# AdeeshKolluru/AdsorbDiff

Hardware: AMD Instinct MI355X
Metric: sampled adsorbate sites/sec (50 denoise steps, ~200-atom slabs) (higher is better)
Workload: dtype f32 (f16x3-split MFMA, fp32 accumulate; ADF_GEMM=f32 selects exact f32)

## Files before the change

### adsorbdiff_amd/csrc/api.hip

```cpp
#include <stdarg.h>
#include <stdlib.h>
#include <string.h>

#include <new>

#include "common.h"

static thread_local char g_err[512] = "";

void adf_set_error(const char* fmt, ...) {
    va_list ap;
    va_start(ap, fmt);
    vsnprintf(g_err, sizeof(g_err), fmt, ap);
    va_end(ap);
}

extern "C" const char* adf_last_error(void) { return g_err; }
extern "C" const char* adf_version(void) { return "adsorbdiff_hip 0.5.0 (gfx950)"; }

adf_tune adf_tune_from_env() {
    auto off_is_0 = [](const char* name) { const char* e = getenv(name); return (e && atoi(e) == 0) ? 0 : 1; };
    auto is_f32 = [](const char* name) { const char* e = getenv(name); return e && strcmp(e, "f32") == 0; };
    adf_tune t = {};
    const char* mi = getenv("ADF_GEMM16_MI");
// ... 5 lines not shown
    t.gemm_wr_fused = wf ? atoi(wf) : 2;
    if (t.gemm_wr_fused != 0 && t.gemm_wr_fused != 4) t.gemm_wr_fused = 2;
    t.head_gate_fused = off_is_0("ADF_HEAD_GATE_FUSED");
    t.lift_emit = off_is_0("ADF_LIFT_EMIT");
    t.graph_sys_csr = off_is_0("ADF_GRAPH_SYS_CSR");
    t.train_gemm16 = is_f32("ADF_TRAIN_GEMM") ? 0 : 1;
    t.wgrad_f32 = is_f32("ADF_WGRAD") ? 1 : 0;
    const char* pw = getenv("ADF_EQV2_PW_MI");
    t.eqv2_pw_mi = (pw && atoi(pw) == 3) ? 3 : 4;
    const char* gt = getenv("ADF_EQV2_GEMM_TILE");
    t.eqv2_gemm_tile256 = (gt && atoi(gt) == 128) ? 0 : 1;
    t.eqv2_rotin_generic = getenv("ADF_EQV2_ROTIN_GENERIC") != nullptr;
    t.eqv2_rotout_generic = getenv("ADF_EQV2_ROTOUT_GENERIC") != nullptr;
    const char* r4 = getenv("ADF_GEMM_ROWS4");
    t.gemm_rows4 = r4 ? (atoi(r4) & 3) : 3;
    return t;
}
const adf_tune& adf_tune_process() {
    static const adf_tune t = adf_tune_from_env();
    return t;
}
int adf_current_num_cus() {
    int dev = 0, n = 0;
    if (hipGetDevice(&dev) != hipSuccess || hipDeviceGetAttribute(&n, hipDeviceAttributeMultiprocessorCount, dev) != hipSuccess) return 0;
    return n;
}

extern "C" int32_t adf_profile_enable(adf_painn_t h, int32_t on) {
    if (!h) { adf_set_error("null handle"); return ADF_EINVAL; }
    h->prof.enable(on != 0);
// ... 377 lines not shown
    const bool lift = h->lift_on && !h->gemm_f32;
    const bool em = lift && h->tune.lift_emit;
    ADF_TRY(adf_nodewise_layernorm(x, w.ln_w, w.ln_b, h->y, n, H, s, em ? h->mag_a : nullptr, h->rows_dev));
    ADF_TRY(adf_linear(h, h->y, H, w.xp0_w, &w.xp0_16, w.xp0_b, h->cat, H, n, H, H, 1, s, em ? h->mag_a : nullptr,
                       em ? h->mag_b : nullptr));
    if (h->gemm_f32) {
        if (row_map) { adf_set_error("internal: mapped records need the f16x3 path"); return ADF_EINVAL; }
        ADF_TRY(adf_launch_gemm(h->cat, H, w.xp2_w, H, w.xp2_b, h->xh, 3 * H, n, 3 * H, H, 0, s));
        ADF_TRY(adf_pack_records(h, n, h->xh, vec, vec_is_zero, s, rec));
    } else {
        adf_epi ep = {};
        ep.vec_in = vec; ep.rec = rec ? rec : h->rec; ep.H = H; ep.vec_is_zero = vec_is_zero ? 1 : 0;
        ep.row_map = row_map;
        ep.rmag = em ? h->mag_b : nullptr;
        ep.m_dev = h->rows_dev;
        ADF_TRY(adf_launch_gemm16_fused(h->cat, H, &w.xp2_16, n, H, H, 1, &ep, s, h->tune, lift ? &h->lift : nullptr));
    }
    adf_prof_end(h, s);
    return ADF_OK;
}

static int32_t message_layer(adf_painn* h, int l, int N, const float* x, const float* vec, float* x_out,
                             float* vec_out, bool vec_is_zero, hipStream_t s, const int32_t* tlist = nullptr,
                             int n_targets = 0, float* rec = nullptr, bool records_ready = false) {
    if (!records_ready) ADF_TRY(make_records(h, l, N, x, vec, vec_is_zero, rec, nullptr, s));
    adf_prof_begin(h, ADF_PROF_MESSAGE, s);
    const int items = tlist ? n_targets : N;
    const bool emit = h->rmx && h->lift_on && !h->gemm_f32 && !h->msg_f32 && items > 0 && items <= h->part_stride;
    h->part_x = h->part_vec = nullptr;
    const int32_t st = adf_message_impl(h, l, N, x, h->xh, vec, x_out, vec_out, vec_is_zero, s, tlist, n_targets, rec,
                                        tlist ? h->rows_dev : nullptr, emit ? h->xpart : nullptr, h->vpart, h->part_stride);
// ... 39 lines not shown
        adf_epi e0 = {};
        e0.A2 = h->cat; e0.K1 = H; e0.m_dev = h->rows_dev;
        e0.rmag = parts ? h->lift.buf : nullptr;
        e0.out_mag = h->lift_on ? reinterpret_cast<unsigned int*>(h->mag_b) : nullptr;
        ADF_TRY(adf_launch_gemm16(x, H, &w.xv0_16, w.xv0_b, h->y, H, N, H, 2 * H, 1, &e0, s, lf, h->tune, h->num_cus));
    }
    int32_t st;
    if (h->gemm_f32) {
        ADF_TRY(adf_launch_gemm(h->y, H, w.xv2_w, H, w.xv2_b, h->xh, 3 * H, N, 3 * H, H, 0, s));
        st = adf_nodewise_update_apply(h->xh, h->dot, h->vv, x, vec, h->scale[l], N, H, s);
    } else {
        adf_epi ep = {};
        ep.x = x; ep.vec = vec; ep.dot = h->dot; ep.vv = h->vv; ep.scale = h->scale[l]; ep.H = H;
        ep.rmag = h->lift_on ? h->mag_b : nullptr;
        ep.m_dev = h->rows_dev;
        st = adf_launch_gemm16_fused(h->y, H, &w.xv2_16, N, H, H, 2, &ep, s, h->tune);
    }
    adf_prof_end(h, s);
    return st;
}

extern "C" int32_t adf_painn_message_layer(adf_painn_t h, int32_t layer, int32_t N, const float* x, const float* vec,
                                           float* x_out, float* vec_out, void* stream) {
    if (!h || !h->weights_set || layer < 0 || layer >= h->hp.num_layers || N != h->lastN) {
        adf_set_error("message_layer: bad handle/layer, or N differs from the built graph");
        return ADF_EINVAL;
    }
    hipStream_t s = (hipStream_t)stream;
    ADF_TRY(zero_pad_rows(h, N, s));
    ADF_TRY(message_layer(h, layer, N, x, vec, x_out, vec_out, false, s));
    return ADF_OK;
}

extern "C" int32_t adf_painn_update_layer(adf_painn_t h, int32_t layer, int32_t N, float* x, float* vec, void* stream) {
    if (!h || !h->weights_set || layer < 0 || layer >= h->hp.num_layers) {
        adf_set_error("update_layer: bad handle/layer");
        return ADF_EINVAL;
    }
    ADF_TRY(ensure_capacity(h, N, 1));
    return update_layer(h, layer, N, x, vec, (hipStream_t)stream, false);
}

extern "C" int32_t adf_painn_get_tune(adf_painn_t h, adf_tune* out) {
    if (!h || !out) { adf_set_error("get_tune: null handle or output"); return ADF_EINVAL; }
    *out = h->tune;
    return ADF_OK;
}

extern "C" int32_t adf_painn_debug_row_maxima(adf_painn_t h, int32_t which, float* out, int64_t capacity, int32_t* rows,
                                              void* stream) {
    if (!h || which < 0 || which > 6) { adf_set_error("debug_row_maxima: null handle or which outside 0..6"); return ADF_EINVAL; }
    if (which == 4) { h->dbg_capture = capacity != 0; h->dbg_comb_rows = 0; return ADF_OK; }
    const int H = h->hp.hidden_channels, ns = H / ADF_SLICE_CH;
    const int n = which <= 1 ? h->dbg_msg_rows : which <= 3 ? h->dbg_cat_rows : h->dbg_comb_rows;
    if (!h->rmx_part || n <= 0) { adf_set_error("debug_row_maxima: no launch has emitted row maxima (ADF_ROW_MAXIMA=0?)"); return ADF_EINVAL; }
    if (rows) *rows = n;
    if (!out) return ADF_OK;
    const int64_t need = (which == 1 || which == 5) ? 3ll * n : which == 3 ? (int64_t)n * H : n;
    if (capacity < need) { adf_set_error("debug_row_maxima: out holds %lld floats, need %lld", (long long)capacity, (long long)need); return ADF_EINVAL; }
    hipStream_t s = (hipStream_t)stream;
// ... 516 lines not shown
```

### adsorbdiff_amd/csrc/common.h

```cpp
#pragma once
#include <hip/hip_runtime.h>
#include <stdint.h>
#include <stdio.h>
#include <string>
#include <vector>

#include "../../include/adsorbdiff_hip.h"

#define ADF_GROUP_NODES 32
#define ADF_SLICE_CH 64
#define ADF_MAX_CAND 1024
#define ADF_MAX_K 128
#define ADF_NFLAGS 8
#define ADF_MAX_INDEG 1024
#define ADF_MAX_LAYERS 16

void adf_set_error(const char* fmt, ...);

#define ADF_HIP_CHECK(expr)                                                             \
    do {                                                                                \
        hipError_t _e = (expr);                                                         \
        if (_e != hipSuccess) {                                                         \
            adf_set_error("%s failed: %s (%s:%d)", #expr, hipGetErrorString(_e),        \
                          __FILE__, __LINE__);                                          \
// ... 260 lines not shown
const adf_tune& adf_tune_process();
int adf_current_num_cus();
int32_t adf_launch_gemm16(const float* A, int lda, const adf_w16* W, const float* bias, float* C, int ldc, int M,
                          int N, int K, int act_ssilu, const adf_epi* ep, hipStream_t s, const adf_lift* lf,
                          const adf_tune& tune, int num_cus);
int32_t adf_launch_rowmag(const float* A, int lda, int K1, const float* A2, int K2, long long M, float* mag, hipStream_t s,
                          const int32_t* m_dev = nullptr, int m_mul = 1);
int32_t adf_launch_rowmax_combine(const float* part, long long stride, int nparts, long long M, float* mag, hipStream_t s,
                                  const int32_t* m_dev = nullptr, int m_mul = 1);
int32_t adf_split_weight(const float* w, long long n, adf_w16* out, unsigned int* scratch_bits, hipStream_t s,
                         int perm_H = 0, int K = 0, const float* bias = nullptr, int parts = 3);
int32_t adf_launch_gemm16_vecnorm(const float* A, int lda, const adf_w16* W, float* nrm, int M, int N, int K,
                                  hipStream_t s, const adf_tune& tune, const adf_lift* lf = nullptr,
                                  const float* premag = nullptr);
int32_t adf_launch_gemm16_fused(const float* A, int lda, const adf_w16* W, int M, int H, int K, int epi,
                                const adf_epi* ep, hipStream_t s, const adf_tune& tune, const adf_lift* lf = nullptr);
static inline int32_t adf_linear(const adf_painn* h, const float* A, int lda, const float* W, const adf_w16* W16,
                                 const float* bias, float* C, int ldc, int M, int N, int K, int act, hipStream_t s,
                                 const float* premag = nullptr, float* out_mag = nullptr) {
    if (h->gemm_f32) return adf_launch_gemm(A, lda, W, K, bias, C, ldc, M, N, K, act, s);
    adf_epi ep = {};
    ep.m_dev = h->rows_dev;
    if (h->lift_on) { ep.rmag = premag; ep.out_mag = reinterpret_cast<unsigned int*>(out_mag); }
    return adf_launch_gemm16(A, lda, W16, bias, C, ldc, M, N, K, act, &ep, s, h->lift_on ? &h->lift : nullptr, h->tune,
                             h->num_cus);
}
int32_t adf_pack_frag(const adf_w16* w, int N, int K, void* out, hipStream_t s);
int32_t adf_graph_build_impl(adf_painn* h, const adf_batch* b, hipStream_t s);
int32_t adf_energy_sum(const float* y, int H2, const float* w, const float* bias, const int32_t* atom_offset, float* energy,
                       int num_systems, hipStream_t s);
__device__ __forceinline__ float adf_row16_max(float v) {
// ... 95 lines not shown
```

### adsorbdiff_amd/csrc/gemm16.hip

```cpp
#include <stdlib.h>

#include "common.h"

typedef float f32x16 __attribute__((ext_vector_type(16)));
typedef _Float16 half8 __attribute__((ext_vector_type(8)));
typedef _Float16 half4 __attribute__((ext_vector_type(4)));

#ifndef EPI_ABL
#define EPI_ABL 0
#endif
#ifndef EPI2_POLICY
#define EPI2_POLICY 0
#endif
#ifndef G16_ABL
#define G16_ABL 0
#endif
#ifndef G16_WDEEP
#define G16_WDEEP 1
#endif
#ifndef G16_START_DELAY
#define G16_START_DELAY 0
#endif
#define HK 32
#define TLD3 96
// ... 2 lines not shown

__device__ __forceinline__ float adf_pow2_lift(float mx) {
    if (!(mx > 0.f) || !(mx < 3.0e38f)) return 1.0f;
    int e;
    (void)frexpf(mx, &e);
    e = 15 - e;
    e = e > 120 ? 120 : (e < -120 ? -120 : e);
    return ldexpf(1.0f, e);
}

__device__ __forceinline__ float ssilu16(float x) {
    float s = x / (1.0f + expf(-x));
    return s * 1.6666666666666667f;
}

template <int ACT, int MI, int NJ, int EPI, bool WR = false, int NWN = 2, int NWM = 2>
__global__ __launch_bounds__(64 * NWM * NWN, (MI == 4 || NWM * NWN == 8 ? 1 : 2)) void adf_gemm_f16x3_kernel(
    const float* __restrict__ A, int lda, const _Float16* __restrict__ Whi, const _Float16* __restrict__ Wlo,
    const float* __restrict__ inv_scale, const float* __restrict__ bias, float* __restrict__ C, int ldc, int Mh, int N,
    int K, int tiles_n, adf_epi ep) {
    const int M = ep.m_dev ? min(Mh, (int)*ep.m_dev) : Mh;
    static_assert(NWN == 2 || WR, "eight waves only with the register-streamed weights");
    static_assert(NWM == 2 || (NWM == 1 && WR), "one wave along M only with the register-streamed weights");
    constexpr int NT = 64 * NWM * NWN;
    constexpr int TM = 32 * MI * NWM;
    constexpr int TN = 32 * NJ * NWN;
    constexpr int NA = TM * 8 / NT;
    static_assert(TM * 8 % NT == 0, "A staging: whole float4s per thread");
    constexpr int LDS_WR = 4 * TM * HLD > NT / 64 * 6400 ? 4 * TM * HLD : NT / 64 * 6400;
    constexpr int LDS_MAIN = WR ? LDS_WR : (2 * TM + 2 * TN) * HLD;
    constexpr int LDS_REC = EPI == 1 ? NT / 64 * 2048 : 0;
    __shared__ __attribute__((aligned(16))) _Float16 lds[LDS_MAIN + LDS_REC];
    __shared__ float rinv[TM];
    _Float16* Ahi = lds;
    _Float16* Alo = Ahi + TM * HLD;
    _Float16* Bhi = Alo + TM * HLD;
    _Float16* Blo = Bhi + TN * HLD;
    const int tid = threadIdx.x;
    const int lane = tid & 63;
    const int wave = tid >> 6;
    const int wm = (wave / NWN) * (32 * MI);
    const int wn = (wave % NWN) * (32 * NJ);

    const int id = blockIdx.x;
    const int xcd = id & 7;
    const int qd = id >> 3;
    const int tile_m = (qd / tiles_n) * 8 + xcd;
    const int tile_n = qd % tiles_n;
    const int m0 = tile_m * (EPI >= 3 ? TM / 3 : TM);
    const int n0 = tile_n * TN;
    if (m0 >= M) return;
#if G16_START_DELAY
    if constexpr (NWM == 1) {
        if (qd >= 32 && qd < 64)
            for (int i = 0; i < G16_START_DELAY; ++i) __builtin_amdgcn_s_sleep(127);
    }
#endif

    unsigned int a_goff[NA];
    int a_off[NA];
    float a_rs[NA];
    auto global_row = [&](int row) -> unsigned int {
        if constexpr (EPI >= 3) {
            const int atom = m0 + (row / 96) * 32 + (row & 31), ax = (row % 96) >> 5;
            return (unsigned int)min(atom, M - 1) * 3u + ax;
        } else {
            return (unsigned int)min(m0 + row, M - 1);
        }
// ... 369 lines not shown
                const float a = acc[0][j][r] * (isc * rinv[wm + lr]), b = acc[1][j][r] * (isc * rinv[wm + 32 + lr]),
                            d = acc[2][j][r] * (isc * rinv[wm + 64 + lr]);
                T[lr * TLD2 + j * 32 + q] = sqrtf(a * a + b * b + d * d);
            }
        }
        __builtin_amdgcn_fence(__ATOMIC_RELEASE, "wavefront");
        __builtin_amdgcn_wave_barrier();
#pragma unroll
        for (int it = 0; it < 8; ++it) {
            const int lr = it * 4 + (lane >> 4), c4 = lane & 15;
            const int n = a0 + lr, c = cb + 4 * c4;
            if (n < M && c < N)
                *reinterpret_cast<float4*>(ep.cat + (size_t)n * N + c) = *reinterpret_cast<const float4*>(T + lr * TLD2 + 4 * c4);
        }
    } else {
        static_assert(EPI >= 3 || (NJ == 3 && MI == 2), "fused epilogues are written for the 64 x 96 wave tile");
        if (((EPI_ABL & 1) && EPI == 1) || ((EPI_ABL & 2) && EPI == 2)) {
            float sacc = 0.f;
            for (int i = 0; i < MI; ++i) for (int j = 0; j < NJ; ++j) for (int r = 0; r < 16; ++r) sacc += acc[i][j][r];
            if (ep.H < 0) ep.x[0] = sacc;
            return;
        }
        const int q = lane & 31;
        const int g = (n0 + wn) / 96;
        const int H = ep.H;
        const float b0 = bias[n0 + wn + q], b1 = bias[n0 + wn + 32 + q], b2 = bias[n0 + wn + 64 + q];
        __syncthreads();
        float* T = reinterpret_cast<float*>(lds) + wave * 3200;
#pragma unroll
        for (int i = 0; i < MI; ++i) {
#pragma unroll
// ... 109 lines not shown
                        for (int ax = 0; ax < 3; ++ax) {
                            float4 t = tv[it][ax];
                            const float4 v1 = w1[it][ax];
                            t.x += p2.x * v1.x; t.y += p2.y * v1.y; t.z += p2.z * v1.z; t.w += p2.w * v1.w;
                            EPI2_ST(rv, vr + ax * H, ep.vec, t);
                        }
                    }
#undef EPI2_ST
                }
            }
            __builtin_amdgcn_wave_barrier();
        }
    }
}

__global__ __launch_bounds__(256) void adf_rowmag_kernel(const float* __restrict__ A, int lda, int K1,
                                                         const float* __restrict__ A2, int K2, long long M,
                                                         float* __restrict__ mag, const int32_t* __restrict__ m_dev,
                                                         int m_mul) {
    const long long r = (long long)blockIdx.x * 4 + (threadIdx.x >> 6);
    const int lane = threadIdx.x & 63;
    if (r >= M || (m_dev && r >= (long long)*m_dev * m_mul)) return;
    float mx = 0.f;
    const float* a = A + (size_t)r * lda;
    for (int k = lane * 4; k < K1; k += 256) {
        const float4 v = *reinterpret_cast<const float4*>(a + k);
        mx = fmaxf(fmaxf(fmaxf(mx, fabsf(v.x)), fabsf(v.y)), fmaxf(fabsf(v.z), fabsf(v.w)));
    }
    if (A2) {
        const float* b = A2 + (size_t)r * lda;
// ... 100 lines not shown
        const long long cs = i >> 7;
        const int s = (int)(cs % nks), cb = (int)(cs / nks);
        const _Float16* src = (plane ? lo : hi) + (size_t)(32 * cb + (lane & 31)) * K + 16 * s + 8 * (lane >> 5);
        out[i] = *reinterpret_cast<const half8*>(src);
    }
}

int32_t adf_pack_frag(const adf_w16* w, int N, int K, void* out, hipStream_t s) {
    if (N % 32 || K % 16) { adf_set_error("pack_frag: N %% 32 or K %% 16"); return ADF_EINVAL; }
    hipLaunchKernelGGL(adf_pack_frag_kernel, dim3(256), dim3(256), 0, s, (const _Float16*)w->hi, (const _Float16*)w->lo,
                       (half8*)out, N, K);
    ADF_HIP_CHECK(hipGetLastError());
    return ADF_OK;
}

static int32_t check_a_span(long long rows, int lda) {
    if (rows * (long long)lda * 4 >= (1ll << 32)) {
        adf_set_error("gemm16: A operand of %lld rows x %d exceeds the 32-bit offset range, split the batch", rows, lda);
        return ADF_EOOM;
    }
    return ADF_OK;
}

int32_t adf_launch_gemm16(const float* A, int lda, const adf_w16* W, const float* bias, float* C, int ldc, int M,
                          int N, int K, int act_ssilu, const adf_epi* ep_in, hipStream_t s, const adf_lift* lf,
                          const adf_tune& tune, int num_cus) {
    if (M <= 0) return ADF_OK;
    adf_epi ep = {};
    if (ep_in) ep = *ep_in;
    if (!ep.A2) ep.K1 = 0;
// ... 7 lines not shown
    const int tiles_n = (N + TN - 1) / TN;
    const int tiles_m = (M + TM - 1) / TM;
    const int tiles_m8 = (tiles_m + 7) / 8 * 8;
    dim3 grid((unsigned)(tiles_m8 * tiles_n));
    if (ep.gate && (((N | ldc | ep.gate_ld) & 3) || (((uintptr_t)C | (uintptr_t)ep.gate) & 15))) {
        adf_set_error("gemm16: the gate epilogue needs N, ldc and gate_ld multiples of 4 and 16-byte aligned C and gate");
        return ADF_EINVAL;
    }
    ADF_TRY(lift_mags(A, lda, ep.A2 ? ep.K1 : K, ep.A2, ep.A2 ? K - ep.K1 : 0, M, lf, ep.rmag, &ep.rmag, s, ep.m_dev, 1));
    if (ep.out_mag) ADF_HIP_CHECK(hipMemsetAsync(ep.out_mag, 0, sizeof(float) * (size_t)M, s));
    const int ncu = num_cus > 0 ? num_cus : 256;
    const long long wg8 = (long long)((M + 191) / 192) * (N / 256 > 0 ? N / 256 : 1);
    const bool ragged = wg8 < 4ll * ncu && wg8 % ncu != 0 && wg8 % ncu < (3 * ncu) / 10 && wg8 > ncu;
    const long long wg4 = (long long)((M + 95) / 96) * (N / 256 > 0 ? N / 256 : 1), slots4 = 2ll * ncu;
    const bool ragged4 = wg4 < 4 * slots4 && wg4 % slots4 != 0 && wg4 % slots4 < (3 * slots4) / 10 && wg4 > slots4;
    if ((tune.gemm_rows4 & 1) && tune.gemm_w8_plain && W->frag && N % 256 == 0 && (K / HK) % 2 == 0 && mi == 2 && !ragged4) {
        const int tn4 = N / 256, tmw4 = ((M + 95) / 96 + 7) / 8 * 8;
        dim3 g4((unsigned)(tmw4 * tn4));
        if (act_ssilu)
            hipLaunchKernelGGL((adf_gemm_f16x3_kernel<1, 3, 2, 0, true, 4, 1>), g4, dim3(256), 0, s, A, lda, (const _Float16*)W->frag,
                               (const _Float16*)nullptr, W->inv_scale, bias, C, ldc, M, N, K, tn4, ep);
        else
            hipLaunchKernelGGL((adf_gemm_f16x3_kernel<0, 3, 2, 0, true, 4, 1>), g4, dim3(256), 0, s, A, lda, (const _Float16*)W->frag,
                               (const _Float16*)nullptr, W->inv_scale, bias, C, ldc, M, N, K, tn4, ep);
        ADF_HIP_CHECK(hipGetLastError());
        return ADF_OK;
    }
    if (!(tune.gemm_rows4 & 1) && tune.gemm_w8_plain && W->frag && N % 256 == 0 && (K / HK) % 2 == 0 && mi == 2 && !ragged) {
        const int tn8 = N / 256, tmw8 = ((M + 191) / 192 + 7) / 8 * 8;
        dim3 g8((unsigned)(tmw8 * tn8));
// ... 37 lines not shown
    if (tune.gemm_w8 && W->frag && N % 256 == 0 && (K / HK) % 2 == 0) {
        hipLaunchKernelGGL((adf_gemm_f16x3_kernel<0, 3, 2, 4, true, 4>), dim3((unsigned)(tm8 * (N / 256))), dim3(512), 0, s, A, lda,
                           (const _Float16*)W->frag, (const _Float16*)nullptr, W->inv_scale, (const float*)nullptr,
                           (float*)nullptr, 0, M, N, K, N / 256, ep);
        ADF_HIP_CHECK(hipGetLastError());
        return ADF_OK;
    }
    hipLaunchKernelGGL((adf_gemm_f16x3_kernel<0, 3, 2, 4>), dim3((unsigned)(tm8 * tn)), dim3(256), 0, s, A, lda,
                       (const _Float16*)W->hi, (const _Float16*)W->lo, W->inv_scale, (const float*)nullptr,
                       (float*)nullptr, 0, M, N, K, tn, ep);
    ADF_HIP_CHECK(hipGetLastError());
    return ADF_OK;
}

int32_t adf_launch_gemm16_fused(const float* A, int lda, const adf_w16* W, int M, int H, int K, int epi,
                                const adf_epi* ep_in, hipStream_t s, const adf_tune& tune, const adf_lift* lf) {
    adf_epi epv = *ep_in;
    const adf_epi* ep = &epv;
    if (M <= 0) return ADF_OK;
    if (K % HK != 0 || (lda & 3) || H % 64 != 0 || (epi != 3 && !W->bias_perm)) {
        adf_set_error("gemm16_fused: bad shape");
        return ADF_EINVAL;
    }
    ADF_TRY(check_a_span(epi == 3 ? 3ll * M : (long long)M, lda));
    ADF_TRY(lift_mags(A, lda, K, nullptr, 0, epi == 3 ? 3ll * M : (long long)M, lf, ep_in->rmag, &epv.rmag, s, ep_in->m_dev,
                      epi == 3 ? 3 : 1));
    const int N = 3 * H, TM = 128, TN = 192;
    const int tiles_n = N / TN;
    const int tiles_m = (M + TM - 1) / TM;
    const int tiles_m8 = (tiles_m + 7) / 8 * 8;
    dim3 grid((unsigned)(tiles_m8 * tiles_n));
// ... 3 lines not shown
            hipLaunchKernelGGL((adf_gemm_f16x3_kernel<0, 3, 2, 3, true, 4, 1>), dim3((unsigned)(((M + 31) / 32 + 7) / 8 * 8 * (2 * H / 256))),
                               dim3(256), 0, s, A, lda, (const _Float16*)W->frag, (const _Float16*)nullptr, W->inv_scale,
                               (const float*)nullptr, (float*)nullptr, 0, M, 2 * H, K, 2 * H / 256, *ep);
        else if (tune.gemm_wreg && W->frag && tune.gemm_w8 && (2 * H) % 256 == 0 && (K / HK) % 2 == 0)
            hipLaunchKernelGGL((adf_gemm_f16x3_kernel<0, 3, 2, 3, true, 4>), dim3((unsigned)(tm8 * (2 * H / 256))), dim3(512), 0, s,
                               A, lda, (const _Float16*)W->frag, (const _Float16*)nullptr, W->inv_scale, (const float*)nullptr,
                               (float*)nullptr, 0, M, 2 * H, K, 2 * H / 256, *ep);
        else
        hipLaunchKernelGGL((adf_gemm_f16x3_kernel<0, 3, 2, 3>), dim3((unsigned)(tm8 * tn)), dim3(256), 0, s, A, lda,
                           (const _Float16*)W->hi, (const _Float16*)W->lo, W->inv_scale, (const float*)nullptr,
                           (float*)nullptr, 0, M, 2 * H, K, tn, *ep);
        ADF_HIP_CHECK(hipGetLastError());
        return ADF_OK;
    }
    const int wf = tune.gemm_wr_fused;
    if ((tune.gemm_rows4 & 2) && wf == 2 && W->frag && (K / HK) % 2 == 0 && N % 384 == 0) {
        dim3 g4((unsigned)(((M + 63) / 64 + 7) / 8 * 8 * (N / 384)));
        if (epi == 1)
            hipLaunchKernelGGL((adf_gemm_f16x3_kernel<0, 2, 3, 1, true, 4, 1>), g4, dim3(256), 0, s, A, lda, (const _Float16*)W->frag,
                               (const _Float16*)nullptr, W->inv_scale, W->bias_perm, (float*)nullptr, 0, M, N, K, N / 384, *ep);
        else
            hipLaunchKernelGGL((adf_gemm_f16x3_kernel<0, 2, 3, 2, true, 4, 1>), g4, dim3(256), 0, s, A, lda, (const _Float16*)W->frag,
                               (const _Float16*)nullptr, W->inv_scale, W->bias_perm, (float*)nullptr, 0, M, N, K, N / 384, *ep);
        ADF_HIP_CHECK(hipGetLastError());
        return ADF_OK;
    }
    if (wf && W->frag && (K / HK) % 2 == 0 && (wf == 2 || N % 384 == 0)) {
        const int tnw = wf == 4 ? N / 384 : tiles_n;
        dim3 gw((unsigned)(tiles_m8 * tnw));
#define LAUNCHWF(EPI_, NWN_)                                                                                                  \
// ... 19 lines not shown
```

### adsorbdiff_amd/lib.py

```python
from __future__ import annotations

import ctypes as C
from pathlib import Path

ADF_OK, ADF_EINVAL, ADF_EOOM, ADF_ENONEIGHBOR, ADF_EHIP, ADF_EOVERFLOW, ADF_ENUMERIC = 0, 1, 2, 3, 4, 5, 6


class NumericRangeError(ArithmeticError):
    """Non-finite model output (ADF_ENUMERIC).  Not a RuntimeError on purpose: ``ml_diffuse`` must not answer it by
    splitting the batch; the engine answers it by re-running in exact f32."""

EXPORTS = (
    "adf_painn_create", "adf_painn_destroy", "adf_painn_set_weights", "adf_graph_build", "adf_graph_set_moving",
    "adf_check_flags", "adf_painn_set_arithmetic", "adf_painn_set_incremental", "adf_painn_get_tune",
    "adf_graph_export", "adf_painn_forward", "adf_painn_forward_subset", "adf_linear_forward", "adf_painn_message_layer", "adf_painn_update_layer",
    "adf_painn_debug_row_maxima",
    "adf_sde_init_placement", "adf_sde_step", "adf_sde_step_scheduled", "adf_sample", "adf_sample_traj",
    "adf_tr_step", "adf_tr_sample", "adf_tr_sample_traj",
    "adf_painn_set_per_system_stop", "adf_eqv2_set_per_system_stop", "adf_sampler_draws",
    "adf_painn_set_energy_head", "adf_painn_set_distance_floor", "adf_painn_forward_energy",
    "adf_painn_forward_energy_gradient", "adf_painn_energy_gradient_workspace",
    "adf_lbfgs_create", "adf_lbfgs_destroy", "adf_lbfgs_reset", "adf_lbfgs_converge", "adf_lbfgs_step",
    "adf_lbfgs_get_mask", "adf_lbfgs_last_step_max", "adf_lbfgs_set_per_system", "adf_lbfgs_get_step_state",
    "adf_lbfgs_active_build", "adf_active_gather", "adf_active_scatter",
    "adf_frames_create", "adf_frames_destroy", "adf_frames_push", "adf_frames_wait", "adf_frames_release", "adf_frames_pushed", "adf_frames_abort",
    "adf_get_counters", "adf_profile_enable", "adf_profile_read", "adf_measure_peaks",
    "adf_lift_adsorbates", "adf_flag_anomalies", "adf_select_best_sites",
    "adf_site_pair_distances", "adf_unique_sites", "adf_select_top_sites",
    "adf_place_draws", "adf_place_adsorbates", "adf_place_site_candidates", "adf_interstitial_distances", "adf_comm_unique_id", "adf_comm_create", "adf_comm_destroy", "adf_allgather_sites",
    "adf_op_linear_fwd", "adf_op_linear_bwd_scratch", "adf_op_linear_bwd", "adf_op_ssilu_fwd", "adf_op_ssilu_bwd", "adf_op_layernorm_fwd", "adf_op_layernorm_bwd", "adf_op_embed_fwd", "adf_op_embed_bwd", "adf_op_rbf", "adf_op_message_fwd", "adf_op_message_fwd_fused", "adf_op_message_bwd", "adf_op_message_bwd_fused", "adf_op_message_bwd_fused_supported", "adf_op_message_bwd_perm", "adf_op_edge_owner", "adf_op_rbf_image_bytes", "adf_op_rbf_image", "adf_op_rbf_wgrad_fused_scratch", "adf_op_rbf_wgrad_fused", "adf_op_vdot_fwd", "adf_op_vdot_bwd", "adf_op_update_out_fwd", "adf_op_update_out_bwd", "adf_op_vnorm_fwd", "adf_op_vnorm_bwd", "adf_op_gate_fwd", "adf_op_gate_bwd", "adf_op_copy_rows", "adf_op_score_loss", "adf_op_score_loss_tr", "adf_op_s2ef_loss", "adf_op_s2ef_loss_scratch", "adf_op_energy_sum", "adf_op_energy_head_bwd", "adf_op_energy_head_bwd_scratch", "adf_op_sqnorm_accumulate", "adf_op_adamw_step",
    "adf_op_optimizer_chunk", "adf_op_grad_sqnorm_multi", "adf_op_adamw_multi", "adf_op_embed_bwd_ordered", "adf_op_embed_bwd_ordered_scratch",
# ... 25 lines not shown
        ("max_neighbors", C.c_int32), ("max_radius", C.c_float), ("avg_degree", C.c_float),
    ]


class EqV2Counters(C.Structure):
    _fields_ = [("num_edges", C.c_int64), ("num_atoms", C.c_int64), ("dense_flops", C.c_int64), ("conv_flops", C.c_int64),
                ("inc_rows", C.c_int64), ("inc_rows_full", C.c_int64), ("forwards_total", C.c_int64),
                ("conv_flops_total", C.c_int64)]


class Tune(C.Structure):
    _fields_ = [(name, C.c_int32) for name in (
        "gemm16_mi", "gemm_w8_plain", "gemm_w8", "gemm_wreg", "gemm_wr_fused", "head_gate_fused", "lift_emit",
        "graph_sys_csr", "train_gemm16", "wgrad_f32",
        "eqv2_pw_mi", "eqv2_gemm_tile256", "eqv2_rotin_generic", "eqv2_rotout_generic",
        "gemm_rows4")]


class BatchDesc(C.Structure):
    _fields_ = [
        ("num_systems", C.c_int32), ("num_atoms", C.c_int32), ("pos", C.c_void_p), ("cell", C.c_void_p),
        ("atomic_numbers", C.c_void_p), ("batch", C.c_void_p), ("atom_offset", C.c_void_p), ("reps", C.c_int32 * 3),
    ]


class ActiveField(C.Structure):
    _fields_ = [("src", C.c_void_p), ("dst", C.c_void_p), ("row_bytes", C.c_int32), ("per_system", C.c_int32)]


class StepCoef(C.Structure):
    _fields_ = [
# ... 46 lines not shown
        "adf_painn_destroy": [vp],
        "adf_painn_set_weights": [vp, i32, C.POINTER(vp), C.POINTER(C.c_float), vp],
        "adf_graph_build": [vp, C.POINTER(BatchDesc), vp, C.POINTER(i64)],
        "adf_graph_set_moving": [vp, vp, vp, vp],
        "adf_check_flags": [vp, vp],
        "adf_painn_set_arithmetic": [vp, i32],
        "adf_painn_set_incremental": [vp, i32],
        "adf_painn_get_tune": [vp, C.POINTER(Tune)],
        "adf_graph_export": [vp, vp, vp, vp, i64, vp, vp, vp, vp, C.POINTER(i64), vp],
        "adf_painn_forward": [vp, C.POINTER(BatchDesc), vp, vp, vp],
        "adf_painn_forward_subset": [vp, C.POINTER(BatchDesc), vp, i32, vp, vp, vp],
        "adf_painn_message_layer": [vp, i32, i32, vp, vp, vp, vp, vp],
        "adf_linear_forward": [vp, vp, vp, vp, i32, i32, i32, i32, i32, vp],
        "adf_painn_update_layer": [vp, i32, i32, vp, vp, vp],
        "adf_painn_debug_row_maxima": [vp, i32, vp, C.c_int64, C.POINTER(i32), vp],
        "adf_sde_init_placement": [vp, C.POINTER(BatchDesc), vp, vp, vp, vp],
        "adf_sde_step": [vp, C.POINTER(BatchDesc), vp, vp, vp, vp, vp, C.POINTER(StepCoef), vp, vp, i32, vp, vp, vp, vp],
        "adf_sde_step_scheduled": [vp, C.POINTER(BatchDesc), vp, vp, vp, vp, vp, vp, i32, vp, vp, i32, vp, vp, vp, vp],
        "adf_tr_step": [vp, C.POINTER(BatchDesc), vp, vp, vp, C.POINTER(TrCoef), vp, i32, vp, i32, vp, vp, vp],
        "adf_tr_sample": [vp, C.POINTER(BatchDesc), vp, vp, vp, i32, vp, i32, i32, vp, vp, i32, vp, vp],
        "adf_tr_sample_traj": [vp, C.POINTER(BatchDesc), vp, vp, vp, i32, vp, i32, i32, vp, vp, i32, vp, vp, i32, vp],
        "adf_eqv2_tr_step": [vp, C.POINTER(BatchDesc), vp, vp, vp, C.POINTER(TrCoef), vp, i32, vp, i32, vp, vp, vp],
        "adf_eqv2_tr_sample": [vp, C.POINTER(BatchDesc), vp, vp, vp, i32, vp, i32, i32, vp, vp, i32, vp, vp],
        "adf_eqv2_tr_sample_traj": [vp, C.POINTER(BatchDesc), vp, vp, vp, i32, vp, i32, i32, vp, vp, i32, vp, vp, i32, vp],
        "adf_painn_set_energy_head": [vp, i32, C.POINTER(vp), vp],
        "adf_painn_set_distance_floor": [vp, C.c_float],
        "adf_painn_forward_energy": [vp, C.POINTER(BatchDesc), vp, vp, vp],
        "adf_painn_forward_energy_gradient": [vp, C.POINTER(BatchDesc), vp, vp, vp],
        "adf_painn_energy_gradient_workspace": [vp, i64, C.POINTER(i64)],
        "adf_lbfgs_create": [i64, i32, i32, C.c_double, C.c_double, C.c_double, i32, C.POINTER(vp)],
# ... 156 lines not shown
```

### include/adsorbdiff_hip.h

```cpp
#ifndef ADSORBDIFF_HIP_H
#define ADSORBDIFF_HIP_H

#include <stdint.h>

#ifdef __cplusplus
extern "C" {
#endif

#define ADF_OK 0
#define ADF_EINVAL 1
#define ADF_EOOM 2
#define ADF_ENONEIGHBOR 3
#define ADF_EHIP 4
#define ADF_EOVERFLOW 5
#define ADF_ENUMERIC 6

typedef struct adf_painn* adf_painn_t;

typedef struct {
    int32_t hidden_channels;
    int32_t num_layers;
    int32_t num_rbf;
    int32_t num_elements;
    int32_t max_neighbors;
// ... 34 lines not shown
    int32_t gemm16_mi;
    int32_t gemm_w8_plain;
    int32_t gemm_w8;
    int32_t gemm_wreg;
    int32_t gemm_wr_fused;
    int32_t head_gate_fused;
    int32_t lift_emit;
    int32_t graph_sys_csr;
    int32_t train_gemm16;
    int32_t wgrad_f32;
    int32_t eqv2_pw_mi;
    int32_t eqv2_gemm_tile256;
    int32_t eqv2_rotin_generic;
    int32_t eqv2_rotout_generic;
    int32_t gemm_rows4;
} adf_tune;
int32_t adf_painn_get_tune(adf_painn_t h, adf_tune* out);

int32_t adf_check_flags(adf_painn_t h, void* stream);

int32_t adf_graph_export(adf_painn_t h, int32_t* nbr_count, int32_t* nbr_src, int32_t* nbr_shift,
                         int64_t edge_capacity, int32_t* edge_src, int32_t* edge_dst, float* edge_dist,
                         float* edge_vec, int64_t* num_edges, void* stream);

int32_t adf_painn_forward(adf_painn_t h, const adf_batch* b, float* f1, float* f2, void* stream);

int32_t adf_painn_forward_subset(adf_painn_t h, const adf_batch* b, const int32_t* out_idx, int32_t n_out, float* f1,
                                 float* f2, void* stream);

int32_t adf_painn_message_layer(adf_painn_t h, int32_t layer, int32_t num_atoms, const float* x,
                                const float* vec, float* x_out, float* vec_out, void* stream);
int32_t adf_painn_update_layer(adf_painn_t h, int32_t layer, int32_t num_atoms, float* x, float* vec,
                               void* stream);
int32_t adf_painn_debug_row_maxima(adf_painn_t h, int32_t which, float* out, int64_t capacity, int32_t* rows,
                                   void* stream);

int32_t adf_linear_forward(const float* A, const float* W, const float* bias, float* C, int32_t M, int32_t N,
                           int32_t K, int32_t act_ssilu, int32_t mode, void* stream);

typedef struct {
    float coef_tr;
    float rot_pre;
    float rot_dt;
    float rot_g2;
    float noise_tr;
    float noise_rot;
} adf_step_coef;

int32_t adf_sde_init_placement(adf_painn_t h, const adf_batch* b, float* pos, const int32_t* tags,
                               const float* noise, void* stream);
// ... 372 lines not shown
```

Before: 263.7.

## Split ragged GEMM tail wave into short row tiles via block plan

New measurement: 263.7 (median of 3 runs). No clear change (+0.0%).

```diff
diff --git a/adsorbdiff_amd/csrc/api.hip b/adsorbdiff_amd/csrc/api.hip
--- a/adsorbdiff_amd/csrc/api.hip
+++ b/adsorbdiff_amd/csrc/api.hip
@@ -43,6 +43,8 @@
     t.eqv2_rotout_generic = getenv("ADF_EQV2_ROTOUT_GENERIC") != nullptr;
     const char* r4 = getenv("ADF_GEMM_ROWS4");
     t.gemm_rows4 = r4 ? (atoi(r4) & 3) : 3;
+    const char* gt2 = getenv("ADF_GEMM_TAIL");
+    t.gemm_tail = gt2 ? (atoi(gt2) > 0 ? atoi(gt2) : 0) : 1;
     return t;
 }
 const adf_tune& adf_tune_process() {
@@ -450,7 +452,7 @@
         ep.row_map = row_map;
         ep.rmag = em ? h->mag_b : nullptr;
         ep.m_dev = h->rows_dev;
-        ADF_TRY(adf_launch_gemm16_fused(h->cat, H, &w.xp2_16, n, H, H, 1, &ep, s, h->tune, lift ? &h->lift : nullptr));
+        ADF_TRY(adf_launch_gemm16_fused(h->cat, H, &w.xp2_16, n, H, H, 1, &ep, s, h->tune, lift ? &h->lift : nullptr, h->num_cus));
     }
     adf_prof_end(h, s);
     return ADF_OK;
@@ -520,7 +522,7 @@
         ep.x = x; ep.vec = vec; ep.dot = h->dot; ep.vv = h->vv; ep.scale = h->scale[l]; ep.H = H;
         ep.rmag = h->lift_on ? h->mag_b : nullptr;
         ep.m_dev = h->rows_dev;
-        st = adf_launch_gemm16_fused(h->y, H, &w.xv2_16, N, H, H, 2, &ep, s, h->tune);
+        st = adf_launch_gemm16_fused(h->y, H, &w.xv2_16, N, H, H, 2, &ep, s, h->tune, nullptr, h->num_cus);
     }
     adf_prof_end(h, s);
     return st;
@@ -550,6 +552,12 @@
 extern "C" int32_t adf_painn_get_tune(adf_painn_t h, adf_tune* out) {
     if (!h || !out) { adf_set_error("get_tune: null handle or output"); return ADF_EINVAL; }
     *out = h->tune;
+    return ADF_OK;
+}
+
+extern "C" int32_t adf_painn_debug_rows_dev(adf_painn_t h, const int32_t* rows_dev) {
+    if (!h) { adf_set_error("debug_rows_dev: null handle"); return ADF_EINVAL; }
+    h->rows_dev = rows_dev;
     return ADF_OK;
 }
 
diff --git a/adsorbdiff_amd/csrc/common.h b/adsorbdiff_amd/csrc/common.h
--- a/adsorbdiff_amd/csrc/common.h
+++ b/adsorbdiff_amd/csrc/common.h
@@ -298,7 +298,8 @@
                                   hipStream_t s, const adf_tune& tune, const adf_lift* lf = nullptr,
                                   const float* premag = nullptr);
 int32_t adf_launch_gemm16_fused(const float* A, int lda, const adf_w16* W, int M, int H, int K, int epi,
-                                const adf_epi* ep, hipStream_t s, const adf_tune& tune, const adf_lift* lf = nullptr);
+                                const adf_epi* ep, hipStream_t s, const adf_tune& tune, const adf_lift* lf = nullptr,
+                                int num_cus = 0);
 static inline int32_t adf_linear(const adf_painn* h, const float* A, int lda, const float* W, const adf_w16* W16,
                                  const float* bias, float* C, int ldc, int M, int N, int K, int act, hipStream_t s,
                                  const float* premag = nullptr, float* out_mag = nullptr) {
diff --git a/adsorbdiff_amd/csrc/gemm16.hip b/adsorbdiff_amd/csrc/gemm16.hip
--- a/adsorbdiff_amd/csrc/gemm16.hip
+++ b/adsorbdiff_amd/csrc/gemm16.hip
@@ -1,6 +1,7 @@
 #include <stdlib.h>
 
 #include "common.h"
+#include "gemm16_plan.h"
 
 typedef float f32x16 __attribute__((ext_vector_type(16)));
 typedef _Float16 half8 __attribute__((ext_vector_type(8)));
@@ -40,12 +41,19 @@
     return s * 1.6666666666666667f;
 }
 
+template <int MI, int NJ, int EPI, bool WR, int NWN, int NWM>
+struct adf_g16_lds {
+    static constexpr int NT = 64 * NWM * NWN, TM = 32 * MI * NWM, TN = 32 * NJ * NWN;
+    static constexpr int LDS_WR = 4 * TM * HLD > NT / 64 * 6400 ? 4 * TM * HLD : NT / 64 * 6400;
+    static constexpr int MAIN = WR ? LDS_WR : (2 * TM + 2 * TN) * HLD;
+    static constexpr int REC = EPI == 1 ? NT / 64 * 2048 : 0;
+};
+
 template <int ACT, int MI, int NJ, int EPI, bool WR = false, int NWN = 2, int NWM = 2>
-__global__ __launch_bounds__(64 * NWM * NWN, (MI == 4 || NWM * NWN == 8 ? 1 : 2)) void adf_gemm_f16x3_kernel(
+__device__ __forceinline__ void adf_gemm_f16x3_body(
     const float* __restrict__ A, int lda, const _Float16* __restrict__ Whi, const _Float16* __restrict__ Wlo,
-    const float* __restrict__ inv_scale, const float* __restrict__ bias, float* __restrict__ C, int ldc, int Mh, int N,
-    int K, int tiles_n, adf_epi ep) {
-    const int M = ep.m_dev ? min(Mh, (int)*ep.m_dev) : Mh;
+    const float* __restrict__ inv_scale, const float* __restrict__ bias, float* __restrict__ C, int ldc, const int M, int N,
+    int K, const adf_epi& ep, const int m0, const int n0, _Float16* const lds, float* const rinv) {
     static_assert(NWN == 2 || WR, "eight waves only with the register-streamed weights");
     static_assert(NWM == 2 || (NWM == 1 && WR), "one wave along M only with the register-streamed weights");
     constexpr int NT = 64 * NWM * NWN;
@@ -53,11 +61,7 @@
     constexpr int TN = 32 * NJ * NWN;
     constexpr int NA = TM * 8 / NT;
     static_assert(TM * 8 % NT == 0, "A staging: whole float4s per thread");
-    constexpr int LDS_WR = 4 * TM * HLD > NT / 64 * 6400 ? 4 * TM * HLD : NT / 64 * 6400;
-    constexpr int LDS_MAIN = WR ? LDS_WR : (2 * TM + 2 * TN) * HLD;
-    constexpr int LDS_REC = EPI == 1 ? NT / 64 * 2048 : 0;
-    __shared__ __attribute__((aligned(16))) _Float16 lds[LDS_MAIN + LDS_REC];
-    __shared__ float rinv[TM];
+    constexpr int LDS_MAIN = adf_g16_lds<MI, NJ, EPI, WR, NWN, NWM>::MAIN;
     _Float16* Ahi = lds;
     _Float16* Alo = Ahi + TM * HLD;
     _Float16* Bhi = Alo + TM * HLD;
@@ -68,16 +72,9 @@
     const int wm = (wave / NWN) * (32 * MI);
     const int wn = (wave % NWN) * (32 * NJ);
 
-    const int id = blockIdx.x;
-    const int xcd = id & 7;
-    const int qd = id >> 3;
-    const int tile_m = (qd / tiles_n) * 8 + xcd;
-    const int tile_n = qd % tiles_n;
-    const int m0 = tile_m * (EPI >= 3 ? TM / 3 : TM);
-    const int n0 = tile_n * TN;
-    if (m0 >= M) return;
 #if G16_START_DELAY
     if constexpr (NWM == 1) {
+        const int qd = blockIdx.x >> 3;
         if (qd >= 32 && qd < 64)
             for (int i = 0; i < G16_START_DELAY; ++i) __builtin_amdgcn_s_sleep(127);
     }
@@ -477,7 +474,7 @@
                 *reinterpret_cast<float4*>(ep.cat + (size_t)n * N + c) = *reinterpret_cast<const float4*>(T + lr * TLD2 + 4 * c4);
         }
     } else {
-        static_assert(EPI >= 3 || (NJ == 3 && MI == 2), "fused epilogues are written for the 64 x 96 wave tile");
+        static_assert(EPI >= 3 || (NJ == 3 && (MI == 2 || (MI == 1 && NWM == 1))), "fused epilogues are written for the 64 x 96 wave tile (32 x 96: the last round's)");
         if (((EPI_ABL & 1) && EPI == 1) || ((EPI_ABL & 2) && EPI == 2)) {
             float sacc = 0.f;
             for (int i = 0; i < MI; ++i) for (int j = 0; j < NJ; ++j) for (int r = 0; r < 16; ++r) sacc += acc[i][j][r];
@@ -617,6 +614,46 @@
     }
 }
 
+template <int ACT, int MI, int NJ, int EPI, bool WR = false, int NWN = 2, int NWM = 2>
+__global__ __launch_bounds__(64 * NWM * NWN, (MI == 4 || NWM * NWN == 8 ? 1 : 2)) void adf_gemm_f16x3_kernel(
+    const float* __restrict__ A, int lda, const _Float16* __restrict__ Whi, const _Float16* __restrict__ Wlo,
+    const float* __restrict__ inv_scale, const float* __restrict__ bias, float* __restrict__ C, int ldc, int Mh, int N,
+    int K, int tiles_n, adf_epi ep) {
+    const int M = ep.m_dev ? min(Mh, (int)*ep.m_dev) : Mh;
+    using L = adf_g16_lds<MI, NJ, EPI, WR, NWN, NWM>;
+    __shared__ __attribute__((aligned(16))) _Float16 lds[L::MAIN + L::REC];
+    __shared__ float rinv[L::TM];
+    const int id = blockIdx.x;
+    const int xcd = id & 7;
+    const int qd = id >> 3;
+    const int tile_m = (qd / tiles_n) * 8 + xcd;
+    const int tile_n = qd % tiles_n;
+    const int m0 = tile_m * (EPI >= 3 ? L::TM / 3 : L::TM);
+    if (m0 >= M) return;
+    adf_gemm_f16x3_body<ACT, MI, NJ, EPI, WR, NWN, NWM>(A, lda, Whi, Wlo, inv_scale, bias, C, ldc, M, N, K, ep, m0, tile_n * L::TN,
+                                                        lds, rinv);
+}
+
+template <int ACT, int MI, int NJ, int EPI>
+__global__ __launch_bounds__(256, 2) void adf_gemm_f16x3_plan_kernel(
+    const float* __restrict__ A, int lda, const _Float16* __restrict__ Wfrag, const float* __restrict__ inv_scale,
+    const float* __restrict__ bias, float* __restrict__ C, int ldc, int Mh, int N, int K, int tiles_n, int slots, adf_epi ep) {
+    const int M = ep.m_dev ? min(Mh, (int)*ep.m_dev) : Mh;
+    using L = adf_g16_lds<MI, NJ, EPI, true, 4, 1>;
+    using LT = adf_g16_lds<1, NJ, EPI, true, 4, 1>;
+    static_assert(L::MAIN + L::REC >= LT::MAIN + LT::REC && L::MAIN == LT::MAIN, "the short tiles live in the long tiles' LDS");
+    __shared__ __attribute__((aligned(16))) _Float16 lds[L::MAIN + L::REC];
+    __shared__ float rinv[L::TM];
+    const adf_g16_tile t = adf_g16_block_tile(adf_g16_make_plan(M, L::TM, LT::TM, tiles_n, slots), (int)blockIdx.x, L::TM, LT::TM, tiles_n);
+    if (t.kind < 0) return;
+    if (t.kind == 0)
+        adf_gemm_f16x3_body<ACT, MI, NJ, EPI, true, 4, 1>(A, lda, Wfrag, nullptr, inv_scale, bias, C, ldc, M, N, K, ep, t.m0,
+                                                          t.tile_n * L::TN, lds, rinv);
+    else
+        adf_gemm_f16x3_body<ACT, 1, NJ, EPI, true, 4, 1>(A, lda, Wfrag, nullptr, inv_scale, bias, C, ldc, M, N, K, ep, t.m0,
+                                                         t.tile_n * LT::TN, lds, rinv);
+}
+
 __global__ __launch_bounds__(256) void adf_rowmag_kernel(const float* __restrict__ A, int lda, int K1,
                                                          const float* __restrict__ A2, int K2, long long M,
                                                          float* __restrict__ mag, const int32_t* __restrict__ m_dev,
@@ -747,6 +784,8 @@
     return ADF_OK;
 }
 
+static int adf_g16_slots(const adf_tune& tune, int ncu) { return tune.gemm_tail > 1 ? tune.gemm_tail : 2 * ncu; }
+
 static int32_t check_a_span(long long rows, int lda) {
     if (rows * (long long)lda * 4 >= (1ll << 32)) {
         adf_set_error("gemm16: A operand of %lld rows x %d exceeds the 32-bit offset range, split the batch", rows, lda);
@@ -784,6 +823,19 @@
     const bool ragged = wg8 < 4ll * ncu && wg8 % ncu != 0 && wg8 % ncu < (3 * ncu) / 10 && wg8 > ncu;
     const long long wg4 = (long long)((M + 95) / 96) * (N / 256 > 0 ? N / 256 : 1), slots4 = 2ll * ncu;
     const bool ragged4 = wg4 < 4 * slots4 && wg4 % slots4 != 0 && wg4 % slots4 < (3 * slots4) / 10 && wg4 > slots4;
+    if (tune.gemm_tail && (tune.gemm_rows4 & 1) && tune.gemm_w8_plain && W->frag && N % 256 == 0 && (K / HK) % 2 == 0 && mi == 2) {
+        const int tn4 = N / 256, slots = adf_g16_slots(tune, ncu);
+        const long long blocks = ep.m_dev ? adf_g16_bound_blocks(M, 96, 32, tn4, slots)
+                                          : adf_g16_plan_blocks(adf_g16_make_plan(M, 96, 32, tn4, slots), tn4);
+        if (act_ssilu)
+            hipLaunchKernelGGL((adf_gemm_f16x3_plan_kernel<1, 3, 2, 0>), dim3((unsigned)blocks), dim3(256), 0, s, A, lda,
+                               (const _Float16*)W->frag, W->inv_scale, bias, C, ldc, M, N, K, tn4, slots, ep);
+        else
+            hipLaunchKernelGGL((adf_gemm_f16x3_plan_kernel<0, 3, 2, 0>), dim3((unsigned)blocks), dim3(256), 0, s, A, lda,
+                               (const _Float16*)W->frag, W->inv_scale, bias, C, ldc, M, N, K, tn4, slots, ep);
+        ADF_HIP_CHECK(hipGetLastError());
+        return ADF_OK;
+    }
     if ((tune.gemm_rows4 & 1) && tune.gemm_w8_plain && W->frag && N % 256 == 0 && (K / HK) % 2 == 0 && mi == 2 && !ragged4) {
         const int tn4 = N / 256, tmw4 = ((M + 95) / 96 + 7) / 8 * 8;
         dim3 g4((unsigned)(tmw4 * tn4));
@@ -851,7 +903,7 @@
 }
 
 int32_t adf_launch_gemm16_fused(const float* A, int lda, const adf_w16* W, int M, int H, int K, int epi,
-                                const adf_epi* ep_in, hipStream_t s, const adf_tune& tune, const adf_lift* lf) {
+                                const adf_epi* ep_in, hipStream_t s, const adf_tune& tune, const adf_lift* lf, int num_cus) {
     adf_epi epv = *ep_in;
     const adf_epi* ep = &epv;
     if (M <= 0) return ADF_OK;
@@ -885,6 +937,19 @@
         return ADF_OK;
     }
     const int wf = tune.gemm_wr_fused;
+    if (tune.gemm_tail && (tune.gemm_rows4 & 2) && wf == 2 && W->frag && (K / HK) % 2 == 0 && N % 384 == 0) {
+        const int tn4 = N / 384, slots = adf_g16_slots(tune, num_cus > 0 ? num_cus : 256);
+        const long long blocks = ep->m_dev ? adf_g16_bound_blocks(M, 64, 32, tn4, slots)
+                                           : adf_g16_plan_blocks(adf_g16_make_plan(M, 64, 32, tn4, slots), tn4);
+        if (epi == 1)
+            hipLaunchKernelGGL((adf_gemm_f16x3_plan_kernel<0, 2, 3, 1>), dim3((unsigned)blocks), dim3(256), 0, s, A, lda,
+                               (const _Float16*)W->frag, W->inv_scale, W->bias_perm, (float*)nullptr, 0, M, N, K, tn4, slots, *ep);
+        else
+            hipLaunchKernelGGL((adf_gemm_f16x3_plan_kernel<0, 2, 3, 2>), dim3((unsigned)blocks), dim3(256), 0, s, A, lda,
+                               (const _Float16*)W->frag, W->inv_scale, W->bias_perm, (float*)nullptr, 0, M, N, K, tn4, slots, *ep);
+        ADF_HIP_CHECK(hipGetLastError());
+        return ADF_OK;
+    }
     if ((tune.gemm_rows4 & 2) && wf == 2 && W->frag && (K / HK) % 2 == 0 && N % 384 == 0) {
         dim3 g4((unsigned)(((M + 63) / 64 + 7) / 8 * 8 * (N / 384)));
         if (epi == 1)
diff --git a/adsorbdiff_amd/csrc/gemm16_plan.h b/adsorbdiff_amd/csrc/gemm16_plan.h
--- /dev/null
+++ b/adsorbdiff_amd/csrc/gemm16_plan.h
@@ -0,0 +1,64 @@
+#pragma once
+
+#if defined(__HIPCC__) || defined(__CUDACC__)
+#define ADF_G16_HD __host__ __device__ inline
+#else
+#define ADF_G16_HD inline
+#endif
+
+struct adf_g16_plan {
+    int main_panels;
+    int tail_panels;
+};
+
+struct adf_g16_tile {
+    int kind;
+    int m0;
+    int tile_n;
+};
+
+ADF_G16_HD adf_g16_plan adf_g16_make_plan(int M, int tm_main, int tm_tail, int tiles_n, int slots) {
+    adf_g16_plan p;
+    p.main_panels = M > 0 ? (M + tm_main - 1) / tm_main : 0;
+    p.tail_panels = 0;
+    const long long wg = (long long)p.main_panels * tiles_n;
+    if (slots <= 0 || wg == 0 || wg % slots == 0) return p;
+    const int full_panels = (int)((wg / slots) * slots / (8ll * tiles_n)) * 8;
+    const int tail = (M - full_panels * tm_main + tm_tail - 1) / tm_tail;
+    if ((long long)tail * tiles_n > slots) return p;
+    p.main_panels = full_panels;
+    p.tail_panels = tail;
+    return p;
+}
+
+ADF_G16_HD long long adf_g16_plan_blocks(adf_g16_plan p, int tiles_n) {
+    return ((long long)(p.main_panels + 7) / 8 * 8 + (long long)(p.tail_panels + 7) / 8 * 8) * tiles_n;
+}
+
+ADF_G16_HD long long adf_g16_bound_blocks(int Mh, int tm_main, int tm_tail, int tiles_n, int slots) {
+    if (Mh <= 0) return 0;
+    const long long panels = (Mh + tm_main - 1) / tm_main;
+    const long long all_main = (panels + 7) / 8 * 8 * tiles_n;
+    if (slots <= 0) return all_main;
+    const long long full_panels = (panels * tiles_n / slots) * slots / (8ll * tiles_n) * 8;
+    long long tail = slots / tiles_n;
+    const long long tail_rows = (Mh + tm_tail - 1) / tm_tail;
+    if (tail > tail_rows) tail = tail_rows;
+    const long long mixed = (full_panels + (tail + 7) / 8 * 8) * tiles_n;
+    return all_main > mixed ? all_main : mixed;
+}
+
+ADF_G16_HD adf_g16_tile adf_g16_block_tile(adf_g16_plan p, int block, int tm_main, int tm_tail, int tiles_n) {
+    adf_g16_tile t;
+    t.kind = -1; t.m0 = 0; t.tile_n = 0;
+    const int main_blocks = (p.main_panels + 7) / 8 * 8 * tiles_n;
+    const int kind = block < main_blocks ? 0 : 1;
+    const int id = kind ? block - main_blocks : block;
+    const int qd = id >> 3;
+    const int panel = (qd / tiles_n) * 8 + (id & 7);
+    if (panel >= (kind ? p.tail_panels : p.main_panels)) return t;
+    t.kind = kind;
+    t.m0 = kind ? p.main_panels * tm_main + panel * tm_tail : panel * tm_main;
+    t.tile_n = qd % tiles_n;
+    return t;
+}
diff --git a/adsorbdiff_amd/lib.py b/adsorbdiff_amd/lib.py
--- a/adsorbdiff_amd/lib.py
+++ b/adsorbdiff_amd/lib.py
@@ -14,7 +14,7 @@
     "adf_painn_create", "adf_painn_destroy", "adf_painn_set_weights", "adf_graph_build", "adf_graph_set_moving",
     "adf_check_flags", "adf_painn_set_arithmetic", "adf_painn_set_incremental", "adf_painn_get_tune",
     "adf_graph_export", "adf_painn_forward", "adf_painn_forward_subset", "adf_linear_forward", "adf_painn_message_layer", "adf_painn_update_layer",
-    "adf_painn_debug_row_maxima",
+    "adf_painn_debug_row_maxima", "adf_painn_debug_rows_dev",
     "adf_sde_init_placement", "adf_sde_step", "adf_sde_step_scheduled", "adf_sample", "adf_sample_traj",
     "adf_tr_step", "adf_tr_sample", "adf_tr_sample_traj",
     "adf_painn_set_per_system_stop", "adf_eqv2_set_per_system_stop", "adf_sampler_draws",
@@ -70,7 +70,7 @@
         "gemm16_mi", "gemm_w8_plain", "gemm_w8", "gemm_wreg", "gemm_wr_fused", "head_gate_fused", "lift_emit",
         "graph_sys_csr", "train_gemm16", "wgrad_f32",
         "eqv2_pw_mi", "eqv2_gemm_tile256", "eqv2_rotin_generic", "eqv2_rotout_generic",
-        "gemm_rows4")]
+        "gemm_rows4", "gemm_tail")]
 
 
 class BatchDesc(C.Structure):
@@ -147,6 +147,7 @@
         "adf_linear_forward": [vp, vp, vp, vp, i32, i32, i32, i32, i32, vp],
         "adf_painn_update_layer": [vp, i32, i32, vp, vp, vp],
         "adf_painn_debug_row_maxima": [vp, i32, vp, C.c_int64, C.POINTER(i32), vp],
+        "adf_painn_debug_rows_dev": [vp, vp],
         "adf_sde_init_placement": [vp, C.POINTER(BatchDesc), vp, vp, vp, vp],
         "adf_sde_step": [vp, C.POINTER(BatchDesc), vp, vp, vp, vp, vp, C.POINTER(StepCoef), vp, vp, i32, vp, vp, vp, vp],
         "adf_sde_step_scheduled": [vp, C.POINTER(BatchDesc), vp, vp, vp, vp, vp, vp, i32, vp, vp, i32, vp, vp, vp, vp],
diff --git a/include/adsorbdiff_hip.h b/include/adsorbdiff_hip.h
--- a/include/adsorbdiff_hip.h
+++ b/include/adsorbdiff_hip.h
@@ -72,6 +72,7 @@
     int32_t eqv2_rotin_generic;
     int32_t eqv2_rotout_generic;
     int32_t gemm_rows4;
+    int32_t gemm_tail;
 } adf_tune;
 int32_t adf_painn_get_tune(adf_painn_t h, adf_tune* out);
 
@@ -92,6 +93,8 @@
                                void* stream);
 int32_t adf_painn_debug_row_maxima(adf_painn_t h, int32_t which, float* out, int64_t capacity, int32_t* rows,
                                    void* stream);
+
+int32_t adf_painn_debug_rows_dev(adf_painn_t h, const int32_t* rows_dev);
 
 int32_t adf_linear_forward(const float* A, const float* W, const float* bias, float* C, int32_t M, int32_t N,
                            int32_t K, int32_t act_ssilu, int32_t mode, void* stream);
```
